# sunbains/scann-rust

Measured on NVIDIA B200. Metric: queries/sec @ recall@10>=0.95 (Tree-AH 10Mx96), higher is better.
Workload: dtype u8 LUT / u32 accumulate, f32 reorder

## Files before the change

scann-rust_b200/csrc/tc_gemm.cu:

```cuda
#include <cuda.h>
#include <cuda_bf16.h>

#include <stdlib.h>

#include <algorithm>

#include "kernels.h"

namespace scann {

namespace {

constexpr int kTcBM = 128;
constexpr int kTcBN = 128;
constexpr int kTcAtomK = 64;
constexpr int kTcAtomBytes = kTcBM * 128;
constexpr int kTcEpiWarps = 16;
constexpr int kTcThreads = 32 * (2 + kTcEpiWarps);
constexpr int kTcTmemCols = 512;
constexpr int kWqLane = 8;
constexpr int kWqFlushAt = 6;
constexpr int kWqBytes = kWqLane * 32 * 8 + 16;

__device__ __forceinline__ uint32_t smem_u32(const void* p) {
// ... 326 lines not shown
  tc_fence_before();
  __syncthreads();
  if (warp == 2) {
    tc_fence_after();
    asm volatile("tcgen05.dealloc.cta_group::1.sync.aligned.b32 %0, %1;" ::"r"(tmem_base), "r"(kTcTmemCols) : "memory");
  }
}

template <bool I8>
__global__ void __launch_bounds__(256) tc_prep_rows_kernel(const void* __restrict__ src, size_t n, size_t dim,
                                                           size_t stride, size_t kpad, size_t rows_pad, float scale,
                                                           int want_norm, __nv_bfloat16* __restrict__ dst,
                                                           float* __restrict__ hx, float* __restrict__ norm_max_key) {
  const size_t r = static_cast<size_t>(blockIdx.x) * 8 + (threadIdx.x >> 5);
  const int lane = threadIdx.x & 31;
  if (r >= rows_pad) return;
  float s = 0.0f;
  for (size_t d = lane; d < kpad; d += 32) {
    float v = 0.0f;
    if (r < n && d < dim)
      v = I8 ? static_cast<float>(static_cast<const int8_t*>(src)[r * stride + d])
             : static_cast<const float*>(src)[r * stride + d];
    dst[r * kpad + d] = __float2bfloat16_rn(v);
    const float f = I8 ? v * scale : v;
    s = fmaf(f, f, s);
  }
#pragma unroll
  for (int o = 16; o > 0; o >>= 1) s += __shfl_xor_sync(0xFFFFFFFFu, s, o);
  if (lane == 0) {
    hx[r] = r < n ? (want_norm ? 0.5f * s : 0.0f) : __int_as_float(0x7F800000);
    if (r < n && norm_max_key) atomicMax(reinterpret_cast<uint32_t*>(norm_max_key), __float_as_uint(s));
  }
}

__global__ void __launch_bounds__(256) tc_prep_queries_kernel(const float* __restrict__ q, size_t nq, size_t dim,
                                                              size_t kpad, size_t q_pad, float scale,
                                                              __nv_bfloat16* __restrict__ dst, float* __restrict__ qn) {
  const size_t r = static_cast<size_t>(blockIdx.x) * 8 + (threadIdx.x >> 5);
  const int lane = threadIdx.x & 31;
  if (r >= q_pad) return;
  float s = 0.0f;
  for (size_t d = lane; d < kpad; d += 32) {
    const float v = (r < nq && d < dim) ? q[r * dim + d] : 0.0f;
    dst[r * kpad + d] = __float2bfloat16_rn(v * scale);
    s = fmaf(v, v, s);
  }
#pragma unroll
  for (int o = 16; o > 0; o >>= 1) s += __shfl_xor_sync(0xFFFFFFFFu, s, o);
  if (lane == 0) qn[r] = s;
}

typedef CUresult (*EncodeTiledFn)(CUtensorMap*, CUtensorMapDataType, cuuint32_t, void*, const cuuint64_t*,
                                  const cuuint64_t*, const cuuint32_t*, const cuuint32_t*, CUtensorMapInterleave,
                                  CUtensorMapSwizzle, CUtensorMapL2promotion, CUtensorMapFloatOOBfill);

EncodeTiledFn encode_fn() {
  static EncodeTiledFn fn = [] {
    void* p = nullptr;
    cudaDriverEntryPointQueryResult qres;
    if (cudaGetDriverEntryPoint("cuTensorMapEncodeTiled", &p, cudaEnableDefault, &qres) != cudaSuccess ||
        qres != cudaDriverEntryPointSuccess)
      p = nullptr;
    return reinterpret_cast<EncodeTiledFn>(p);
  }();
  return fn;
}

scann_status make_map(CUtensorMap* map, const void* base, size_t rows, size_t kpad) {
  EncodeTiledFn fn = encode_fn();
  SCANN_REQUIRE(fn != nullptr, SCANN_UNAVAILABLE, "cuTensorMapEncodeTiled is not available in this driver");
  cuuint64_t dims[2] = {kpad, rows};
  cuuint64_t strides[1] = {kpad * 2};
  cuuint32_t box[2] = {kTcAtomK, kTcBM};
  cuuint32_t estr[2] = {1, 1};
  CUresult r = fn(map, CU_TENSOR_MAP_DATA_TYPE_BFLOAT16, 2, const_cast<void*>(base), dims, strides, box, estr,
                  CU_TENSOR_MAP_INTERLEAVE_NONE, CU_TENSOR_MAP_SWIZZLE_128B, CU_TENSOR_MAP_L2_PROMOTION_L2_256B,
                  CU_TENSOR_MAP_FLOAT_OOB_FILL_NONE);
  SCANN_REQUIRE(r == CUDA_SUCCESS, SCANN_INTERNAL, "cuTensorMapEncodeTiled failed (%d)", static_cast<int>(r));
  return SCANN_OK;
}

}

scann_status tc_make_map_u8(void* map, const void* base, size_t rows, size_t row_bytes) {
  EncodeTiledFn fn = encode_fn();
  SCANN_REQUIRE(fn != nullptr, SCANN_UNAVAILABLE, "cuTensorMapEncodeTiled is not available in this driver");
  cuuint64_t dims[2] = {row_bytes, rows};
  cuuint64_t strides[1] = {row_bytes};
  cuuint32_t box[2] = {128, 128};
  cuuint32_t estr[2] = {1, 1};
  CUresult r = fn(static_cast<CUtensorMap*>(map), CU_TENSOR_MAP_DATA_TYPE_UINT8, 2, const_cast<void*>(base), dims,
                  strides, box, estr, CU_TENSOR_MAP_INTERLEAVE_NONE, CU_TENSOR_MAP_SWIZZLE_128B,
                  CU_TENSOR_MAP_L2_PROMOTION_L2_256B, CU_TENSOR_MAP_FLOAT_OOB_FILL_NONE);
  SCANN_REQUIRE(r == CUDA_SUCCESS, SCANN_INTERNAL, "cuTensorMapEncodeTiled(u8) failed (%d)", static_cast<int>(r));
  return SCANN_OK;
}

namespace {

template <int MT, int KA>
scann_status launch_tc(const CUtensorMap& tmA, const CUtensorMap& tmB, const TcArgs& a, int sms, cudaStream_t s) {
  constexpr int kBudget = 225 * 1024 - kTcEpiWarps * kWqBytes;
  constexpr int kStagesRaw = (kBudget - MT * KA * kTcAtomBytes) / (KA * kTcAtomBytes);
  constexpr int STAGES = kStagesRaw > 6 ? 6 : kStagesRaw;
  static_assert(STAGES >= 2, "operand tiles do not fit");
  const size_t smem = 1024 + static_cast<size_t>(MT + STAGES) * KA * kTcAtomBytes + (2 * STAGES + 6) * 8 + 16 +
                      kTcEpiWarps * kWqBytes;
  auto kern = tc_score_kernel<MT, KA, STAGES>;
  SCANN_CUDA(cudaFuncSetAttribute(kern, cudaFuncAttributeMaxDynamicSharedMemorySize, static_cast<int>(smem)));
  const uint32_t total = a.q_tiles * a.n_units;
  const unsigned grid = static_cast<unsigned>(std::min<uint32_t>(total, static_cast<uint32_t>(sms)));
  kern<<<grid, kTcThreads, smem, s>>>(tmA, tmB, a);
  SCANN_CUDA(cudaGetLastError());
  return SCANN_OK;
}

}

size_t tc_kpad(size_t dim) { return (dim + kTcAtomK - 1) / kTcAtomK * kTcAtomK; }
bool tc_supported(size_t dim) { return dim >= 1 && tc_kpad(dim) <= 256; }
size_t tc_rows_pad(size_t n) { return (n + kTcBN - 1) / kTcBN * kTcBN; }
size_t tc_queries_pad(size_t nq, size_t dim) {
  const size_t m = (tc_kpad(dim) <= 128 ? 2 : 1) * kTcBM;
  return (nq + m - 1) / m * m;
}

scann_status tc_prepare_rows(const void* rows, bool i8, size_t n, size_t dim, size_t stride, float scale,
                             bool want_norm, void* dst_bf16, float* hx, float* norm_max, cudaStream_t s) {
  const size_t kpad = tc_kpad(dim), rows_pad = tc_rows_pad(n);
  if (rows_pad == 0) return SCANN_OK;
  if (norm_max) SCANN_CUDA(cudaMemsetAsync(norm_max, 0, sizeof(float), s));
  const unsigned grid = static_cast<unsigned>((rows_pad + 7) / 8);
  if (i8)
    tc_prep_rows_kernel<true><<<grid, 256, 0, s>>>(rows, n, dim, stride, kpad, rows_pad, scale, want_norm ? 1 : 0,
                                                   static_cast<__nv_bfloat16*>(dst_bf16), hx, norm_max);
  else
    tc_prep_rows_kernel<false><<<grid, 256, 0, s>>>(rows, n, dim, stride, kpad, rows_pad, scale, want_norm ? 1 : 0,
                                                    static_cast<__nv_bfloat16*>(dst_bf16), hx, norm_max);
  SCANN_CUDA(cudaGetLastError());
  return SCANN_OK;
}

scann_status tc_prepare_queries(const float* q, size_t nq, size_t dim, float scale, void* dst_bf16, float* qn,
                                cudaStream_t s) {
  const size_t kpad = tc_kpad(dim), q_pad = tc_queries_pad(nq, dim);
  if (q_pad == 0) return SCANN_OK;
  tc_prep_queries_kernel<<<static_cast<unsigned>((q_pad + 7) / 8), 256, 0, s>>>(
      q, nq, dim, kpad, q_pad, scale, static_cast<__nv_bfloat16*>(dst_bf16), qn);
  SCANN_CUDA(cudaGetLastError());
  return SCANN_OK;
}

scann_status launch_tc_scores(const TcScoreParams& p, cudaStream_t s) {
  SCANN_REQUIRE(tc_supported(p.dim), SCANN_INVALID_ARGUMENT, "dimension %zu too large for the tensor-core path", p.dim);
  SCANN_REQUIRE(p.row0 % kTcBN == 0, SCANN_INTERNAL, "row0 must be a multiple of %d", kTcBN);
  if (p.nq == 0 || p.nrows == 0) return SCANN_OK;
  const size_t kpad = tc_kpad(p.dim);
  const int ka = static_cast<int>(kpad / kTcAtomK);
  const int mt = ka <= 2 ? 2 : 1;
  CUtensorMap tmA, tmB;
  SCANN_TRY(make_map(&tmA, p.q_bf16, tc_queries_pad(p.nq, p.dim), kpad));
  SCANN_TRY(make_map(&tmB, p.rows_bf16, p.rows_pad_total, kpad));
  TcArgs a;
  a.nq = static_cast<uint32_t>(p.nq);
  a.q_tiles = static_cast<uint32_t>(tc_queries_pad(p.nq, p.dim) / (mt * kTcBM));
  a.row0 = static_cast<uint32_t>(p.row0);
  a.n_tiles = static_cast<uint32_t>((p.nrows + kTcBN - 1) / kTcBN);
  a.tile_stride = static_cast<uint32_t>(p.tile_stride < 1 ? 1 : p.tile_stride);
  uint32_t want_units = static_cast<uint32_t>(std::max(1, 4 * p.sms / static_cast<int>(a.q_tiles)));
  uint32_t tpu = (a.n_tiles + want_units - 1) / want_units;
  if (tpu < 8) {
    const uint32_t t8 = std::min<uint32_t>(8, a.n_tiles);
// ... 92 lines not shown
```

scann-rust_b200/csrc/tcscan.cu:

```cuda
#include <cuda.h>

#include <stdlib.h>
#include <string.h>

#include <algorithm>

#include "kernels.h"
#include "lut16_scan_kernel.cuh"
#include "tcscan.h"

namespace scann {

namespace {

constexpr int ts_threads(int EG) { return 32 * (4 + 4 * EG + 8); }
constexpr int kTsRing = 8;
constexpr int kTsHalf = kTsRing / 2;
constexpr int kTsAcol = 256;
constexpr int kTsAtom = 128 * 128;
constexpr uint32_t kTsBig = 32768;
constexpr uint32_t kNoKey = 0xFFFFFFFFu;

__device__ __forceinline__ uint32_t smem_u32(const void* p) {
  return static_cast<uint32_t>(__cvta_generic_to_shared(p));
}
__device__ __forceinline__ void mbar_init(uint32_t bar, uint32_t count) {
  asm volatile("mbarrier.init.shared::cta.b64 [%0], %1;" ::"r"(bar), "r"(count));
}
__device__ __forceinline__ void mbar_expect_tx(uint32_t bar, uint32_t bytes) {
  asm volatile("mbarrier.arrive.expect_tx.shared::cta.b64 _, [%0], %1;" ::"r"(bar), "r"(bytes) : "memory");
}
__device__ __forceinline__ void mbar_arrive(uint32_t bar) {
  asm volatile("mbarrier.arrive.shared::cta.b64 _, [%0];" ::"r"(bar) : "memory");
}
__device__ volatile uint32_t* g_tcs_dbg = nullptr;
__device__ __forceinline__ void dbg_mark(int idx, uint32_t v) {
  volatile uint32_t* d = g_tcs_dbg;
  if (d != nullptr && blockIdx.x == 0) d[8 + idx] = v;
}
__device__ __forceinline__ void mbar_wait(uint32_t bar, uint32_t parity, uint32_t tag = 0) {
  uint32_t ok = 0;
  for (uint32_t it = 0; !ok; ++it) {
    asm volatile(
        "{\n\t.reg .pred p;\n\tmbarrier.try_wait.parity.shared::cta.b64 p, [%1], %2;\n\tselp.u32 %0, 1, 0, p;\n\t}"
        : "=r"(ok)
        : "r"(bar), "r"(parity)
        : "memory");
    if (!ok && it > (1u << 22)) {
      volatile uint32_t* d = g_tcs_dbg;
      if (d != nullptr && atomicCAS(const_cast<uint32_t*>(d), 0u, 1u) == 0u) {
        d[1] = bar;
        d[2] = parity;
        d[3] = tag;
        d[4] = blockIdx.x;
        d[5] = threadIdx.x;
        __threadfence_system();
      }
      __trap();
    }
  }
}
__device__ __forceinline__ void tma_load_2d(uint32_t dst, const CUtensorMap* map, uint32_t bar, int c0, int c1) {
  asm volatile(
      "cp.async.bulk.tensor.2d.shared::cluster.global.mbarrier::complete_tx::bytes [%0], [%1, {%3, %4}], [%2];" ::"r"(dst),
      "l"(map), "r"(bar), "r"(c0), "r"(c1)
      : "memory");
}
__device__ __forceinline__ void tc_fence_before() { asm volatile("tcgen05.fence::before_thread_sync;" ::: "memory"); }
__device__ __forceinline__ void tc_fence_after() { asm volatile("tcgen05.fence::after_thread_sync;" ::: "memory"); }
__device__ __forceinline__ void tc_commit(uint32_t bar) {
  asm volatile("tcgen05.commit.cta_group::1.mbarrier::arrive::one.shared::cluster.b64 [%0];" ::"r"(bar) : "memory");
}
__device__ __forceinline__ void mma_i8_ts(uint32_t d, uint32_t a_tmem, uint64_t bdesc, uint32_t idesc, uint32_t acc) {
  asm volatile(
      "{\n\t.reg .pred p;\n\tsetp.ne.b32 p, %4, 0;\n\t"
      "tcgen05.mma.cta_group::1.kind::i8 [%0], [%1], %2, %3, p;\n\t}" ::"r"(d),
      "r"(a_tmem), "l"(bdesc), "r"(idesc), "r"(acc)
      : "memory");
}
__device__ __forceinline__ void tc_ld32(uint32_t taddr, uint32_t (&v)[32]) {
  asm volatile(
      "tcgen05.ld.sync.aligned.32x32b.x32.b32 "
      "{%0, %1, %2, %3, %4, %5, %6, %7, %8, %9, %10, %11, %12, %13, %14, %15, "
      "%16, %17, %18, %19, %20, %21, %22, %23, %24, %25, %26, %27, %28, %29, %30, %31}, [%32];"
      : "=r"(v[0]), "=r"(v[1]), "=r"(v[2]), "=r"(v[3]), "=r"(v[4]), "=r"(v[5]), "=r"(v[6]), "=r"(v[7]), "=r"(v[8]),
        "=r"(v[9]), "=r"(v[10]), "=r"(v[11]), "=r"(v[12]), "=r"(v[13]), "=r"(v[14]), "=r"(v[15]), "=r"(v[16]),
        "=r"(v[17]), "=r"(v[18]), "=r"(v[19]), "=r"(v[20]), "=r"(v[21]), "=r"(v[22]), "=r"(v[23]), "=r"(v[24]),
        "=r"(v[25]), "=r"(v[26]), "=r"(v[27]), "=r"(v[28]), "=r"(v[29]), "=r"(v[30]), "=r"(v[31])
      : "r"(taddr)
      : "memory");
  asm volatile("tcgen05.wait::ld.sync.aligned;" ::: "memory");
}
__device__ __forceinline__ void tc_ld32_nowait(uint32_t taddr, uint32_t (&v)[32]) {
  asm volatile(
      "tcgen05.ld.sync.aligned.32x32b.x32.b32 "
      "{%0, %1, %2, %3, %4, %5, %6, %7, %8, %9, %10, %11, %12, %13, %14, %15, "
      "%16, %17, %18, %19, %20, %21, %22, %23, %24, %25, %26, %27, %28, %29, %30, %31}, [%32];"
      : "=r"(v[0]), "=r"(v[1]), "=r"(v[2]), "=r"(v[3]), "=r"(v[4]), "=r"(v[5]), "=r"(v[6]), "=r"(v[7]), "=r"(v[8]),
        "=r"(v[9]), "=r"(v[10]), "=r"(v[11]), "=r"(v[12]), "=r"(v[13]), "=r"(v[14]), "=r"(v[15]), "=r"(v[16]),
        "=r"(v[17]), "=r"(v[18]), "=r"(v[19]), "=r"(v[20]), "=r"(v[21]), "=r"(v[22]), "=r"(v[23]), "=r"(v[24]),
        "=r"(v[25]), "=r"(v[26]), "=r"(v[27]), "=r"(v[28]), "=r"(v[29]), "=r"(v[30]), "=r"(v[31])
      : "r"(taddr)
      : "memory");
}
__device__ __forceinline__ void tc_wait_ld() { asm volatile("tcgen05.wait::ld.sync.aligned;" ::: "memory"); }
__device__ __forceinline__ void tc_st32(uint32_t taddr, const uint32_t (&v)[32]) {
  asm volatile(
      "tcgen05.st.sync.aligned.32x32b.x32.b32 [%0], "
      "{%1, %2, %3, %4, %5, %6, %7, %8, %9, %10, %11, %12, %13, %14, %15, %16, "
      "%17, %18, %19, %20, %21, %22, %23, %24, %25, %26, %27, %28, %29, %30, %31, %32};" ::"r"(taddr),
      "r"(v[0]), "r"(v[1]), "r"(v[2]), "r"(v[3]), "r"(v[4]), "r"(v[5]), "r"(v[6]), "r"(v[7]), "r"(v[8]), "r"(v[9]),
      "r"(v[10]), "r"(v[11]), "r"(v[12]), "r"(v[13]), "r"(v[14]), "r"(v[15]), "r"(v[16]), "r"(v[17]), "r"(v[18]),
      "r"(v[19]), "r"(v[20]), "r"(v[21]), "r"(v[22]), "r"(v[23]), "r"(v[24]), "r"(v[25]), "r"(v[26]), "r"(v[27]),
      "r"(v[28]), "r"(v[29]), "r"(v[30]), "r"(v[31])
      : "memory");
}
__device__ __forceinline__ void tc_st8(uint32_t taddr, uint32_t v0) {
  const uint32_t z = 0;
  asm volatile("tcgen05.st.sync.aligned.32x32b.x8.b32 [%0], {%1, %2, %3, %4, %5, %6, %7, %8};" ::"r"(taddr), "r"(v0),
               "r"(z), "r"(z), "r"(z), "r"(z), "r"(z), "r"(z), "r"(z)
               : "memory");
}
__device__ __forceinline__ void tc_wait_st() { asm volatile("tcgen05.wait::st.sync.aligned;" ::: "memory"); }
__device__ __forceinline__ uint64_t umma_desc(uint32_t saddr) {
  return static_cast<uint64_t>((saddr >> 4) & 0x3FFFu) | (1ull << 16) | (64ull << 32) | (1ull << 46) | (2ull << 61);
}
__device__ __forceinline__ uint32_t elect_one() {
  uint32_t pred;
  asm volatile("{\n\t.reg .pred P;\n\telect.sync _|P, 0xFFFFFFFF;\n\tselp.u32 %0, 1, 0, P;\n\t}" : "=r"(pred));
  return pred;
}
__device__ __forceinline__ uint32_t shl_clamp(uint32_t v, uint32_t sh) {
  uint32_t r;
  asm("shl.b32 %0, %1, %2;" : "=r"(r) : "r"(v), "r"(sh));
  return r;
}

struct ExpandMul {
  uint32_t sh[8];
  uint32_t eight;
};
__device__ __forceinline__ void expand_onehot(uint32_t C, uint32_t (&r)[32], const ExpandMul& xm) {
#pragma unroll
  for (int i = 0; i < 8; ++i) {
    uint32_t x, t, t1, t2, t3;
    asm("mul.lo.u32 %0, %1, %2;" : "=r"(x) : "r"(C), "r"(xm.sh[i]));
    const uint32_t nib = x >> 28;
    asm("mul.lo.u32 %0, %1, %2;" : "=r"(t) : "r"(nib), "r"(xm.eight));
    asm("mad.lo.u32 %0, %1, %2, 0xFFFFFFE0;" : "=r"(t1) : "r"(nib), "r"(xm.eight));
    asm("mad.lo.u32 %0, %1, %2, 0xFFFFFFC0;" : "=r"(t2) : "r"(nib), "r"(xm.eight));
    asm("mad.lo.u32 %0, %1, %2, 0xFFFFFFA0;" : "=r"(t3) : "r"(nib), "r"(xm.eight));
    r[4 * i + 0] = shl_clamp(1u, t);
    r[4 * i + 1] = shl_clamp(1u, t1);
    r[4 * i + 2] = shl_clamp(1u, t2);
    r[4 * i + 3] = shl_clamp(1u, t3);
  }
}

__device__ __forceinline__ int score_bound_from_tau(float tau, float mult, float biasS, int smax_all) {
  const float est = __fdiv_rn(__fsub_rn(tau, biasS), mult);
  long long s;
  if (!(est == est)) return -2;
  if (est < -1.0f) s = -1;
  else if (est > static_cast<float>(smax_all)) s = smax_all;
  else s = static_cast<long long>(floorf(est));
  for (int it = 0; it < 8 && s < smax_all && lut16_dequant(static_cast<uint32_t>(s + 1), mult, biasS) <= tau; ++it) ++s;
  for (int it = 0; it < 8 && s >= 0 && lut16_dequant(static_cast<uint32_t>(s), mult, biasS) > tau; --s, ++it) {
  }
  if (s >= 0 && lut16_dequant(static_cast<uint32_t>(s), mult, biasS) > tau) return -2;
  if (s < smax_all && lut16_dequant(static_cast<uint32_t>(s + 1), mult, biasS) <= tau) return -2;
  return static_cast<int>(s);
}

__global__ void tcwl_count_kernel(const uint32_t* __restrict__ tokens, size_t P, uint32_t K, uint32_t L, uint32_t T,
                                  const uint64_t* __restrict__ pt_off, uint32_t* __restrict__ leaf_cnt) {
  const size_t p = static_cast<size_t>(blockIdx.x) * blockDim.x + threadIdx.x;
  if (p >= P || static_cast<uint32_t>(p) % L < T) return;
  const uint32_t leaf = tokens[p];
  if (leaf < K && pt_off[leaf + 1] > pt_off[leaf]) atomicAdd(&leaf_cnt[leaf], 1u);
}

__device__ __forceinline__ void tcwl_entry(uint32_t leaf, const uint32_t* __restrict__ leaf_cnt,
                                           const uint64_t* __restrict__ pt_off, uint32_t& pc, uint32_t& groups,
                                           uint32_t& chunks) {
// ... 4 lines not shown
}

__global__ void __launch_bounds__(1024) tcwl_scan_kernel(const uint32_t* __restrict__ leaf_cnt, uint32_t K,
                                                         const uint32_t* __restrict__ perm,
                                                         const uint64_t* __restrict__ pt_off,
                                                         uint32_t* __restrict__ pair_start,
                                                         uint32_t* __restrict__ group_start,
                                                         uint32_t* __restrict__ item_start,
                                                         uint32_t* __restrict__ counters,
                                                         unsigned long long* __restrict__ pair_points) {
  __shared__ uint32_t s_p[1024], s_g[1024], s_i[1024];
  unsigned long long pp_local = 0;
  const uint32_t per = (K + 1023) / 1024;
  const uint32_t b = threadIdx.x * per, e = min(K, b + per);
  uint32_t sp = 0, sg = 0, si = 0;
  for (uint32_t i = b; i < e; ++i) {
    uint32_t pc, g, c;
    tcwl_entry(perm[i], leaf_cnt, pt_off, pc, g, c);
    sp += pc;
    sg += g;
    si += g * c;
    pp_local += static_cast<unsigned long long>(pc) * (pt_off[perm[i] + 1] - pt_off[perm[i]]);
  }
  if (pair_points && pp_local) atomicAdd(pair_points, pp_local);
  s_p[threadIdx.x] = sp;
  s_g[threadIdx.x] = sg;
  s_i[threadIdx.x] = si;
  __syncthreads();
  for (int o = 1; o < 1024; o <<= 1) {
    uint32_t vp = 0, vg = 0, vi = 0;
    if (threadIdx.x >= o) {
      vp = s_p[threadIdx.x - o];
      vg = s_g[threadIdx.x - o];
      vi = s_i[threadIdx.x - o];
    }
    __syncthreads();
    s_p[threadIdx.x] += vp;
    s_g[threadIdx.x] += vg;
    s_i[threadIdx.x] += vi;
    __syncthreads();
  }
  uint32_t rp = s_p[threadIdx.x] - sp, rg = s_g[threadIdx.x] - sg, ri = s_i[threadIdx.x] - si;
  for (uint32_t i = b; i < e; ++i) {
    const uint32_t leaf = perm[i];
    uint32_t pc, g, c;
    tcwl_entry(leaf, leaf_cnt, pt_off, pc, g, c);
    pair_start[leaf] = rp;
    group_start[leaf] = rg;
    item_start[leaf] = ri;
    rp += pc;
    rg += g;
    ri += g * c;
  }
  if (threadIdx.x == 1023) {
    counters[0] = s_i[1023];
    counters[1] = s_g[1023];
    counters[2] = 0;
  }
}

__global__ void tcwl_scatter_kernel(const uint32_t* __restrict__ tokens, size_t P, uint32_t K, uint32_t L, uint32_t T,
                                    const uint64_t* __restrict__ pt_off, const uint32_t* __restrict__ pair_start,
                                    uint32_t* __restrict__ cursor, uint32_t* __restrict__ sorted_pairs) {
  const size_t p = static_cast<size_t>(blockIdx.x) * blockDim.x + threadIdx.x;
  if (p >= P || static_cast<uint32_t>(p) % L < T) return;
  const uint32_t leaf = tokens[p];
  if (leaf < K && pt_off[leaf + 1] > pt_off[leaf])
    sorted_pairs[pair_start[leaf] + atomicAdd(&cursor[leaf], 1u)] = static_cast<uint32_t>(p);
}

__global__ void tcwl_items_kernel(const uint32_t* __restrict__ leaf_cnt, uint32_t K,
                                  const uint64_t* __restrict__ pt_off, const uint32_t* __restrict__ pair_start,
                                  const uint32_t* __restrict__ group_start, const uint32_t* __restrict__ item_start,
                                  uint4* __restrict__ groups, uint4* __restrict__ items) {
  const uint32_t leaf = blockIdx.x * blockDim.x + threadIdx.x;
  if (leaf >= K) return;
  uint32_t pc, ng, nc;
  tcwl_entry(leaf, leaf_cnt, pt_off, pc, ng, nc);
  if (pc == 0) return;
  const uint32_t tiles = static_cast<uint32_t>((pt_off[leaf + 1] - pt_off[leaf] + kTcsTile - 1) / kTcsTile);
  const uint32_t per = (tiles + nc - 1) / nc;
  const uint32_t pb = pair_start[leaf], gb = group_start[leaf], ib = item_start[leaf];
  for (uint32_t g = 0; g < ng; ++g) {
    groups[gb + g] = make_uint4(leaf, pb + g * kTcsGroup, min(static_cast<uint32_t>(kTcsGroup), pc - g * kTcsGroup), 0u);
    for (uint32_t c = 0; c < nc; ++c)
      items[ib + g * nc + c] = make_uint4(gb + g, c * per, min(tiles, (c + 1) * per), leaf);
  }
}

struct LutArgs {
  const uint4* groups;
  const uint32_t* counters;
  const uint32_t* sorted_pairs;
  const float* queries;
  const float* centers;
  const float* codebook;
  const uint32_t* qthr;
  uint8_t* lut;
  uint4* meta;
  uint32_t* qflag;
  int dim, S, ds, L, use_residuals, row_bytes;
};

__device__ __forceinline__ uint32_t lut16_quantize_nonneg(float v, float mn, float scale) {
  const float y = __fmul_rn(__fsub_rn(v, mn), scale);
  uint32_t i = __float2uint_rd(y);
  i += __fsub_rn(y, __uint2float_rn(i)) >= 0.5f ? 1u : 0u;
  return min(i, 255u);
}

template <int DS>
__global__ void __launch_bounds__(256, DS > 0 ? 4 : 2) tc_lut_kernel(const LutArgs a) {
  extern __shared__ __align__(16) uint8_t sm[];
  const int warp = threadIdx.x >> 5, lane = threadIdx.x & 31;
  float* qres = reinterpret_cast<float*>(sm) + warp * a.dim;
  const int nstep = a.S / 8;
  constexpr int kDs = DS > 0 ? DS : 1;
  float* cbs = reinterpret_cast<float*>(sm) + 8 * a.dim;
  if (DS > 0) {
    for (int i = threadIdx.x; i < a.S * 16 * DS; i += blockDim.x) cbs[i] = __ldg(a.codebook + i);
    __syncthreads();
  }
  const uint32_t ngroups = a.counters[1];
  const uint32_t total = ngroups * kTcsGroup;
  for (uint32_t r = blockIdx.x * 8 + warp; r < total; r += gridDim.x * 8) {
    const uint32_t g = r / kTcsGroup, j = r % kTcsGroup;
    const uint4 G = a.groups[g];
    const uint32_t ncol = (G.z + 15u) & ~15u;
    if (j >= ncol) continue;
    uint8_t* out = a.lut + static_cast<size_t>(r) * a.row_bytes;
    uint32_t val = kTsBig + 1u;
    float mult = 1.0f, biasS = 0.0f;
    uint32_t pair = kNoKey;
    if (j < G.z) {
      pair = a.sorted_pairs[G.y + j];
      const uint32_t q = pair / static_cast<uint32_t>(a.L);
      __syncwarp();
      for (int d = lane; d < a.dim; d += 32) {
        float v = a.queries[static_cast<size_t>(q) * a.dim + d];
        if (a.use_residuals) v = __fsub_rn(v, __ldg(a.centers + static_cast<size_t>(G.x) * a.dim + d));
        qres[d] = v;
      }
      __syncwarp();
      float vals[8][4];
      float mn = 3.402823466e+38f, mx = -3.402823466e+38f;
#pragma unroll
      for (int t = 0; t < 8; ++t) {
        if (t < nstep) {
          const int s = 8 * t + (lane >> 2);
          float cw[4 * kDs];
          if (DS > 0) {
            const float4* c4 = reinterpret_cast<const float4*>(cbs + (128 * t + 4 * lane) * DS);
#pragma unroll
            for (int v = 0; v < kDs; ++v) {
              const float4 x = c4[v];
              cw[4 * v + 0] = x.x;
              cw[4 * v + 1] = x.y;
              cw[4 * v + 2] = x.z;
              cw[4 * v + 3] = x.w;
            }
          }
#pragma unroll
          for (int b = 0; b < 4; ++b) {
            float sum = 0.0f;
            if (DS > 0) {
#pragma unroll
              for (int jj = 0; jj < kDs; ++jj) {
// ... 22 lines not shown
      }
#pragma unroll
      for (int t = 0; t < 8; ++t) {
        if (t < nstep) {
          const uint32_t w = lut16_quantize_nonneg(vals[t][0], mn, scale) | (lut16_quantize_nonneg(vals[t][1], mn, scale) << 8) |
                             (lut16_quantize_nonneg(vals[t][2], mn, scale) << 16) |
                             (lut16_quantize_nonneg(vals[t][3], mn, scale) << 24);
          reinterpret_cast<uint32_t*>(out)[32 * t + lane] = w;
        }
      }
      biasS = __fmul_rn(mn, static_cast<float>(a.S));
      const uint32_t tk = a.qthr[q];
      int sb = -2;
      if (tk != kNoKey) sb = score_bound_from_tau(key_f32(tk), mult, biasS, 255 * a.S);
      if (sb == -2) {
        if (lane == 0) a.qflag[q] = 1u;
      } else {
        val = kTsBig - static_cast<uint32_t>(sb);
      }
    } else {
      for (int v = lane; v < a.S; v += 32) reinterpret_cast<uint4*>(out)[v] = make_uint4(0, 0, 0, 0);
    }
    if (lane < 2) {
      uint4 t = make_uint4(0, 0, 0, 0);
      if (lane == 0) t.x = (val % 255u) | ((val / 255u) << 8);
      reinterpret_cast<uint4*>(out + a.S * 16)[lane] = t;
    }
    if (lane == 0) a.meta[r] = make_uint4(__float_as_uint(mult), __float_as_uint(biasS), val, pair);
  }
}

struct TcsArgs {
  const uint8_t* codes_rm;
  const uint64_t* pt_off;
  const uint4* groups;
  const uint4* items;
  const uint32_t* counters;
  const uint4* meta;
  unsigned long long* qcand;
  uint32_t* qcnt;
  uint32_t* err;
  uint32_t qcap;
  uint32_t nq;
  ExpandMul xm;
  int KA;
  int bpp;
  int L;
};

struct TcsFilter {
  const uint8_t* allow;
  size_t allow_stride;
  const uint32_t* qfilt;
  const uint32_t* blk_off;
  uint32_t num_filters;
};

template <bool FILT>
__device__ __forceinline__ void tcs_emit(const TcsArgs& a, const TcsFilter& f, uint32_t lut_row, uint32_t acc, uint32_t pos,
                                         uint32_t leaf) {
  const uint4 m = __ldg(a.meta + lut_row);
  const uint32_t q = m.w / static_cast<uint32_t>(a.L), rank = m.w - q * static_cast<uint32_t>(a.L);
  if (m.w == kNoKey || q >= a.nq) {
    atomicAdd(a.err, 1u);
    return;
  }
  if (FILT) {
    const uint32_t row = f.qfilt ? __ldg(f.qfilt + q) : 0u;
    if (row >= f.num_filters) return;
    const size_t at = row * f.allow_stride + (static_cast<size_t>(__ldg(f.blk_off + leaf)) + (pos >> 8)) * 32 +
                      ((pos & 255u) >> 3);
    if (!((__ldg(f.allow + at) >> (pos & 7u)) & 1u)) return;
  }
  const uint32_t sum = acc - m.z;
  const float dist = lut16_dequant(sum, __uint_as_float(m.x), __uint_as_float(m.y));
  const uint32_t slot = atomicAdd(a.qcnt + q, 1u);
  if (slot < a.qcap)
    a.qcand[static_cast<size_t>(q) * a.qcap + slot] =
        (static_cast<unsigned long long>(f32_key(dist)) << 32) | (static_cast<unsigned long long>(rank) << 22) | pos;
}

constexpr int kWqCap = 320;
constexpr int kWqStep = 256;

template <int EG, bool FILT>
__global__ void __launch_bounds__(ts_threads(EG), 1) tc_scan_kernel(const __grid_constant__ CUtensorMap tmB, const TcsArgs a,
                                                                    const TcsFilter filt) {
  extern __shared__ uint8_t smem_raw[];
  uint8_t* smem = reinterpret_cast<uint8_t*>((reinterpret_cast<uintptr_t>(smem_raw) + 1023) & ~uintptr_t(1023));
  uint8_t* sB = smem;
  uint64_t* bars = reinterpret_cast<uint64_t*>(sB + (a.KA + 1) * kTsAtom);
  constexpr int kBFull = 0, kBEmpty = 1, kAFull = 2, kAEmpty = 2 + kTsRing, kTFull = 2 + 2 * kTsRing,
                kTEmpty = 4 + 2 * kTsRing, kNumBars = 6 + 2 * kTsRing;
  uint32_t* tmem_slot = reinterpret_cast<uint32_t*>(bars + kNumBars);
  uint4* wq_base = reinterpret_cast<uint4*>(tmem_slot + 4);
  uint32_t* wq_cnt_base = reinterpret_cast<uint32_t*>(wq_base + 8 * kWqCap);
  const int warp = threadIdx.x >> 5, lane = threadIdx.x & 31;
  const uint32_t bar0 = smem_u32(bars);
  auto bar = [&](int i) { return bar0 + 8u * static_cast<uint32_t>(i); };

  if (warp == 0 && lane == 0) asm volatile("prefetch.tensormap [%0];" ::"l"(&tmB) : "memory");
  if (warp == 1 && lane == 0) {
    mbar_init(bar(kBFull), 1);
    mbar_init(bar(kBEmpty), 2);
    for (int i = 0; i < kTsRing; ++i) {
      mbar_init(bar(kAFull + i), 4);
      mbar_init(bar(kAEmpty + i), 1);
    }
    for (int i = 0; i < 2; ++i) {
      mbar_init(bar(kTFull + i), 1);
      mbar_init(bar(kTEmpty + i), 8);
    }
    asm volatile("fence.mbarrier_init.release.cluster;" ::: "memory");
  }
  if (warp == 3) {
    asm volatile("tcgen05.alloc.cta_group::1.sync.aligned.shared::cta.b32 [%0], %1;" ::"r"(smem_u32(tmem_slot)), "r"(512)
                 : "memory");
    asm volatile("tcgen05.relinquish_alloc_permit.cta_group::1.sync.aligned;" ::: "memory");
  }
  tc_fence_before();
  __syncthreads();
  tc_fence_after();
  const uint32_t tmem = *tmem_slot;
  const uint32_t n_items = a.counters[0];
  const int nchunk = a.KA + 1;

  if (warp == 0) {
    if (lane == 0) {
      uint32_t it = 0;
      for (uint32_t item = blockIdx.x; item < n_items; item += gridDim.x, ++it) {
        const uint4 I = a.items[item];
        mbar_wait(bar(kBEmpty), (it & 1u) ^ 1u, 0x100u + it);
        mbar_expect_tx(bar(kBFull), static_cast<uint32_t>(nchunk) * kTsAtom);
        for (int c = 0; c < nchunk; ++c)
          tma_load_2d(smem_u32(sB + c * kTsAtom), &tmB, bar(kBFull), c * 128, static_cast<int>(I.x * kTcsGroup));
      }
    }
  } else if (warp == 1 || warp == 2) {
    const uint32_t pp = warp == 1 ? 0u : 1u;
    if (elect_one()) {
      uint32_t it = 0, ts = 0;
      const uint64_t bd0 = umma_desc(smem_u32(sB));
      const uint32_t d = tmem + pp * kTcsGroup;
      const uint32_t a0 = tmem + kTsAcol + pp * kTsHalf * 32;
      for (uint32_t item = blockIdx.x; item < n_items; item += gridDim.x, ++it) {
        const uint4 I = a.items[item];
        const uint32_t ncol = (a.groups[I.x].z + 15u) & ~15u;
        const uint32_t idesc = (2u << 4) | ((ncol >> 3) << 17) | ((128u >> 4) << 24);
        mbar_wait(bar(kBFull), it & 1u, 0x200u + it);
        for (uint32_t t = I.y; t < I.z; ++t, ++ts) {
          if ((ts & 1u) != pp) continue;
          const uint32_t k = ts >> 1;
          mbar_wait(bar(kTEmpty + pp), (k & 1u) ^ 1u, 0x300000u + ts);
          tc_fence_after();
          uint32_t m = k * static_cast<uint32_t>(nchunk);
          for (int c = 0; c < a.KA; ++c, ++m) {
            const uint32_t sl = m % kTsHalf;
            mbar_wait(bar(kAFull + pp * kTsHalf + sl), (m / kTsHalf) & 1u, 0x400000u + m);
            tc_fence_after();
            const uint64_t bd = bd0 + static_cast<uint64_t>(c) * (kTsAtom >> 4);
            const uint32_t at = a0 + sl * 32;
            mma_i8_ts(d, at, bd, idesc, c != 0 ? 1u : 0u);
            mma_i8_ts(d, at + 8, bd + 2u, idesc, 1u);
            mma_i8_ts(d, at + 16, bd + 4u, idesc, 1u);
            mma_i8_ts(d, at + 24, bd + 6u, idesc, 1u);
            tc_commit(bar(kAEmpty + pp * kTsHalf + sl));
// ... 52 lines not shown
          const uint32_t m = m0 + c;
          if (c < a.KA && (EG == 2 || (m & 1u) == sg)) {
            const uint32_t slot = pp * kTsHalf + (m % kTsHalf);
            uint32_t r[32];
            expand_onehot(w[c], r, a.xm);
            publish();
            mbar_wait(bar(kAEmpty + slot), ((m / kTsHalf) & 1u) ^ 1u, 0x500000u + m);
            tc_fence_after();
            tc_st32(tmem + lane_addr + kTsAcol + slot * 32, r);
            prev_slot = static_cast<int>(slot);
          }
        }
        {
          const uint32_t m = m0 + static_cast<uint32_t>(a.KA);
          if (EG == 2 || (m & 1u) == sg) {
            const uint32_t slot = pp * kTsHalf + (m % kTsHalf);
            publish();
            mbar_wait(bar(kAEmpty + slot), ((m / kTsHalf) & 1u) ^ 1u, 0x600000u + m);
            tc_fence_after();
            tc_st8(tmem + lane_addr + kTsAcol + slot * 32, 0x0000FF01u);
            prev_slot = static_cast<int>(slot);
          }
          publish();
        }
      }
    }
  } else if (warp >= 4 + 4 * EG) {
    const uint32_t ew = static_cast<uint32_t>(warp - (4 + 4 * EG));
    const uint32_t half_id = ew >> 2;
    const uint32_t quad = warp & 3;
    const uint32_t row = quad * 32 + lane;
    const uint32_t lane_addr = (quad * 32) << 16;
    uint4* const wq = wq_base + ew * kWqCap;
    volatile uint32_t* const wq_cnt = wq_cnt_base + ew;
    if (lane == 0) *wq_cnt = 0;
    __syncwarp();
    auto flush = [&]() {
      __syncwarp();
      const uint32_t nw = *wq_cnt;
      for (uint32_t i = lane; i < nw; i += 32) {
        const uint4 e = wq[i];
        tcs_emit<FILT>(a, filt, e.x, e.y, e.z, FILT ? e.w : 0u);
      }
      __syncwarp();
      if (lane == 0) *wq_cnt = 0;
      __syncwarp();
    };
    auto filter32 = [&](const uint32_t (&v)[32], uint32_t c0, uint32_t nlive, bool valid, uint32_t lut_row0, uint32_t p,
                        uint32_t leaf) {
      uint32_t m8[4];
#pragma unroll
      for (int g8 = 0; g8 < 4; ++g8) {
        uint32_t m = v[8 * g8];
#pragma unroll
        for (int j = 1; j < 8; ++j) m = min(m, v[8 * g8 + j]);
        m8[g8] = m;
      }
      if (nlive < 32) m8[2] = m8[3] = kNoKey;
      const uint32_t mall = min(min(m8[0], m8[1]), min(m8[2], m8[3]));
      if (__any_sync(0xFFFFFFFFu, valid && mall <= kTsBig)) {
#pragma unroll
        for (int g8 = 0; g8 < 4; ++g8) {
          const bool hit = valid && m8[g8] <= kTsBig;
          if (__any_sync(0xFFFFFFFFu, hit)) {
            if (*wq_cnt > kWqCap - kWqStep) flush();
            if (hit) {
#pragma unroll
              for (int j = 0; j < 8; ++j)
                if (v[8 * g8 + j] <= kTsBig)
                  wq[atomicAdd(const_cast<uint32_t*>(wq_cnt), 1u)] =
                      make_uint4(lut_row0 + c0 + 8 * g8 + j, v[8 * g8 + j], p, FILT ? leaf : 0u);
            }
            __syncwarp();
          }
        }
      }
    };
    uint32_t ts = 0;
    for (uint32_t item = blockIdx.x; item < n_items; item += gridDim.x) {
      const uint4 I = a.items[item];
      const uint32_t ncol = (a.groups[I.x].z + 15u) & ~15u;
      const uint32_t leaf_n = static_cast<uint32_t>(a.pt_off[I.w + 1] - a.pt_off[I.w]);
      const uint32_t lut_row0 = I.x * kTcsGroup;
      const uint32_t cb = half_id * 64;
      const uint32_t nmine = ncol > cb ? min(64u, ncol - cb) : 0u;
      for (uint32_t t = I.y; t < I.z; ++t, ++ts) {
        const uint32_t as = ts & 1u;
        const uint32_t p = t * kTcsTile + row;
        const bool valid = p < leaf_n;
        mbar_wait(bar(kTFull + as), (ts >> 1) & 1u, 0x700000u + ts);
        tc_fence_after();
        const uint32_t taddr = tmem + lane_addr + as * kTcsGroup + cb;
        uint32_t v0[32];
        if (nmine > 0) {
          tc_ld32_nowait(taddr, v0);
          tc_wait_ld();
        }
        if (nmine <= 32) {
          tc_fence_before();
          __syncwarp();
          if (lane == 0) mbar_arrive(bar(kTEmpty + as));
        }
        if (nmine > 0) filter32(v0, cb, min(32u, nmine), valid, lut_row0, p, I.w);
        if (nmine > 32) {
          tc_ld32_nowait(taddr + 32, v0);
          tc_wait_ld();
          tc_fence_before();
          __syncwarp();
          if (lane == 0) mbar_arrive(bar(kTEmpty + as));
          filter32(v0, cb + 32, nmine - 32, valid, lut_row0, p, I.w);
        }
      }
    }
    flush();
  }

  tc_fence_before();
  __syncthreads();
  if (warp == 3) {
    tc_fence_after();
    asm volatile("tcgen05.dealloc.cta_group::1.sync.aligned.b32 %0, %1;" ::"r"(tmem), "r"(512) : "memory");
  }
}

__global__ void tcs_flag_kernel(const uint32_t* __restrict__ tokens, size_t P, uint32_t L, uint32_t T,
                                const uint32_t* __restrict__ qcnt, uint32_t qcap, uint32_t* __restrict__ qflag,
                                uint32_t* __restrict__ fb_tokens) {
  const size_t p = static_cast<size_t>(blockIdx.x) * blockDim.x + threadIdx.x;
  if (p >= P) return;
  const uint32_t p32 = static_cast<uint32_t>(p);
  const uint32_t q = p32 / L, rank = p32 - q * L;
  const bool f = qflag[q] != 0u || qcnt[q] > qcap;
  fb_tokens[p] = (f && rank >= T) ? tokens[p] : kNoKey;
  if (f && rank == 0) qflag[q] = 1u;
}

__global__ void tcs_debug_kernel(const uint32_t* __restrict__ qcnt, const uint32_t* __restrict__ qflag, size_t nq,
                                 uint32_t qcap, unsigned long long* __restrict__ out ) {
  const size_t q = static_cast<size_t>(blockIdx.x) * blockDim.x + threadIdx.x;
  if (q >= nq) return;
  atomicAdd(&out[0], static_cast<unsigned long long>(qcnt[q]));
  atomicMax(&out[1], static_cast<unsigned long long>(qcnt[q]));
  if (qflag[q]) atomicAdd(&out[2], 1ull);
  if (qcnt[q] > qcap) atomicAdd(&out[3], 1ull);
}

}

bool tc_scan_supported(size_t S, size_t dim) {
  return S >= 8 && S <= 64 && S % 8 == 0 && (S / 8) % 2 == 0 && dim % S == 0 && dim * 4 * 8 + S * 16 * 8 <= 48 * 1024;
}

size_t tc_scan_max_groups(size_t P, size_t K) { return P / kTcsGroup + std::min(K, P) + 1; }

size_t tc_scan_max_items(size_t P, size_t K, size_t max_leaf) {
  const size_t tiles = (max_leaf + kTcsTile - 1) / kTcsTile;
  return tc_scan_max_groups(P, K) * std::max<size_t>(1, (tiles + kTcsItemTiles - 1) / kTcsItemTiles);
}

size_t tc_scan_workspace_bytes(size_t nq, size_t L, size_t K, size_t S, size_t max_leaf, size_t qcap) {
  const size_t P = nq * L, G = tc_scan_max_groups(P, K);
  size_t b = 0;
  auto add = [&](size_t bytes) { b += Workspace::padded(bytes); };
  add(2 * K * 4);
  add(3 * (K + 1) * 4);
  add(16);
  add(P * 4);
  add(G * 16);
  add(tc_scan_max_items(P, K, max_leaf) * 16);
  add(G * kTcsGroup * (S * 16 + 32));
  add(G * kTcsGroup * 16);
  add(nq * qcap * 8);
  add(nq * 4);
  add(nq * 4);
  add(P * 4);
  return b + 4096;
}

scann_status launch_tc_scan(const TcScanParams& p, Workspace& ws, TcScanOut* out, cudaStream_t s) {
  const size_t K = p.K, P = p.nq * p.L, S = p.S;
  const size_t G = tc_scan_max_groups(P, K), I = tc_scan_max_items(P, K, p.max_leaf);
  const int row_bytes = static_cast<int>(S * 16 + 32);
  uint32_t* leaf_cnt = ws.take<uint32_t>(2 * K);
  uint32_t* cursor = leaf_cnt + K;
  uint32_t* starts = ws.take<uint32_t>(3 * (K + 1));
  uint32_t *pair_start = starts, *group_start = starts + (K + 1), *item_start = starts + 2 * (K + 1);
  uint32_t* counters = ws.take<uint32_t>(4);
  uint32_t* sorted_pairs = ws.take<uint32_t>(P);
  uint4* groups = ws.take<uint4>(G);
  uint4* items = ws.take<uint4>(I);
  uint8_t* lut = ws.take<uint8_t>(G * kTcsGroup * row_bytes);
  uint4* meta = ws.take<uint4>(G * kTcsGroup);
  unsigned long long* qcand = ws.take<unsigned long long>(p.nq * p.qcap);
  uint32_t* qcnt = ws.take<uint32_t>(p.nq);
  uint32_t* qflag = ws.take<uint32_t>(p.nq);
  uint32_t* fb_tokens = ws.take<uint32_t>(P);

  const char* dbg_env = getenv("SCANN_TC_DEBUG");
  const bool dbg = dbg_env && dbg_env[0] == '1';
  cudaEvent_t ev[5];
  if (dbg)
    for (auto& e : ev) cudaEventCreate(&e);
  if (dbg) cudaEventRecord(ev[0], s);
  SCANN_CUDA(cudaMemsetAsync(qcnt, 0, p.nq * 4, s));
  SCANN_CUDA(cudaMemsetAsync(qflag, 0, p.nq * 4, s));
  const unsigned pb = static_cast<unsigned>((P + 255) / 256);
  const bool reuse = p.wl_cnt != nullptr && p.wl_pair_start != nullptr && p.wl_sorted_pairs != nullptr;
  const uint32_t* cnt_in = leaf_cnt;
  const uint32_t* pairs_in = sorted_pairs;
  if (reuse) {
    cnt_in = p.wl_cnt;
    pairs_in = p.wl_sorted_pairs;
  } else {
    SCANN_CUDA(cudaMemsetAsync(leaf_cnt, 0, 2 * K * 4, s));
    tcwl_count_kernel<<<pb, 256, 0, s>>>(p.tokens, P, static_cast<uint32_t>(K), static_cast<uint32_t>(p.L),
                                         static_cast<uint32_t>(p.T), p.pt_off, leaf_cnt);
  }
  tcwl_scan_kernel<<<1, 1024, 0, s>>>(cnt_in, static_cast<uint32_t>(K), p.leaf_perm, p.pt_off, pair_start, group_start,
                                      item_start, counters, p.pair_points);
  if (!reuse)
    tcwl_scatter_kernel<<<pb, 256, 0, s>>>(p.tokens, P, static_cast<uint32_t>(K), static_cast<uint32_t>(p.L),
                                           static_cast<uint32_t>(p.T), p.pt_off, pair_start, cursor, sorted_pairs);
  tcwl_items_kernel<<<static_cast<unsigned>((K + 127) / 128), 128, 0, s>>>(cnt_in, static_cast<uint32_t>(K), p.pt_off,
                                                                          reuse ? p.wl_pair_start : pair_start,
                                                                          group_start, item_start, groups, items);
  if (dbg) cudaEventRecord(ev[1], s);
  if (p.ev[0]) cudaEventRecord(p.ev[0], s);
  LutArgs la;
  la.groups = groups;
  la.counters = counters;
  la.sorted_pairs = pairs_in;
  la.queries = p.queries;
  la.centers = p.centers;
  la.codebook = p.codebook;
  la.qthr = p.qthr;
  la.lut = lut;
  la.meta = meta;
  la.qflag = qflag;
  la.dim = static_cast<int>(p.dim);
  la.S = static_cast<int>(S);
  la.ds = static_cast<int>(p.dim / S);
  la.L = static_cast<int>(p.L);
  la.use_residuals = p.use_residuals;
  la.row_bytes = row_bytes;
  const size_t lsm = 8 * p.dim * sizeof(float) + (la.ds <= 2 ? S * 16 * la.ds * sizeof(float) : 0);
  const unsigned lgrid = static_cast<unsigned>(p.sms * (la.ds <= 2 ? 4 : 2));
  if (la.ds == 1) tc_lut_kernel<1><<<lgrid, 256, lsm, s>>>(la);
  else if (la.ds == 2) tc_lut_kernel<2><<<lgrid, 256, lsm, s>>>(la);
  else tc_lut_kernel<0><<<lgrid, 256, lsm, s>>>(la);
  SCANN_CUDA(cudaGetLastError());

  if (dbg) cudaEventRecord(ev[2], s);
  if (p.ev[1]) cudaEventRecord(p.ev[1], s);
  alignas(64) CUtensorMap tmB;
  SCANN_TRY(tc_make_map_u8(&tmB, lut, G * kTcsGroup, static_cast<size_t>(row_bytes)));
  TcsArgs a;
  a.codes_rm = p.codes_rm;
  a.pt_off = p.pt_off;
  a.groups = groups;
  a.items = items;
  a.counters = counters;
  a.meta = meta;
  a.qcand = qcand;
  a.qcnt = qcnt;
  a.qcap = static_cast<uint32_t>(p.qcap);
  a.nq = static_cast<uint32_t>(p.nq);
  a.err = counters + 2;
  for (int i = 0; i < 8; ++i) a.xm.sh[i] = 1u << (28 - 4 * i);
  a.xm.eight = 8u;
  a.KA = static_cast<int>(S / 8);
  a.bpp = static_cast<int>(S / 2);
  a.L = static_cast<int>(p.L);
  TcsFilter tf;
  tf.allow = p.allow;
  tf.allow_stride = p.allow_stride;
  tf.qfilt = p.qfilt;
  tf.blk_off = p.blk_off;
  tf.num_filters = p.num_filters;
  const bool filt = p.allow != nullptr;
  const size_t smem = std::max<size_t>(120 * 1024, 1024 + static_cast<size_t>(a.KA + 1) * kTsAtom + 32 * 8 + 64 +
                                                       8 * kWqCap * 16 + 64);
  const char* eg_env = getenv("SCANN_TC_EXP");
  const bool eg4 = eg_env && eg_env[0] == '4';
  auto kern = eg4 ? (filt ? tc_scan_kernel<4, true> : tc_scan_kernel<4, false>)
                  : (filt ? tc_scan_kernel<2, true> : tc_scan_kernel<2, false>);
  SCANN_CUDA(cudaFuncSetAttribute(kern, cudaFuncAttributeMaxDynamicSharedMemorySize, static_cast<int>(smem)));
  static uint32_t* h_dbg = nullptr;
  if (dbg && h_dbg == nullptr) {
    uint32_t* d_dbg = nullptr;
    if (cudaHostAlloc(&h_dbg, 64 * 4, cudaHostAllocMapped) == cudaSuccess &&
        cudaHostGetDevicePointer(&d_dbg, h_dbg, 0) == cudaSuccess) {
      memset(h_dbg, 0, 64 * 4);
      cudaMemcpyToSymbol(g_tcs_dbg, &d_dbg, sizeof(d_dbg));
    }
  }
  kern<<<p.sms, ts_threads(eg4 ? 4 : 2), smem, s>>>(tmB, a, tf);
  SCANN_CUDA(cudaGetLastError());
  if (dbg) {
    cudaError_t e = cudaStreamSynchronize(s);
    if (e != cudaSuccess && h_dbg)
    {
      fprintf(stderr, "[tcscan] scan kernel failed (%s): timed-out wait = %u, barrier smem 0x%x, parity %u, tag 0x%x, cta %u, thread %u\n",
              cudaGetErrorString(e), h_dbg[0], h_dbg[1], h_dbg[2], h_dbg[3], h_dbg[4], h_dbg[5]);
      fprintf(stderr, "[tcscan] cta 0 progress marks (warp: value):");
      for (int w = 0; w < 14; ++w) fprintf(stderr, " %d:0x%x", w, h_dbg[8 + w]);
      fprintf(stderr, "\n");
    }
  }
  if (dbg) cudaEventRecord(ev[3], s);
  if (p.ev[2]) cudaEventRecord(p.ev[2], s);
  tcs_flag_kernel<<<pb, 256, 0, s>>>(p.tokens, P, static_cast<uint32_t>(p.L), static_cast<uint32_t>(p.T), qcnt,
                                     static_cast<uint32_t>(p.qcap), qflag, fb_tokens);
  SCANN_CUDA(cudaGetLastError());
  if (dbg) {
    cudaEventRecord(ev[4], s);
    unsigned long long* d_st = nullptr;
    unsigned long long st[4] = {0, 0, 0, 0};
    uint32_t cnt[3] = {0, 0, 0};
    cudaMalloc(&d_st, sizeof(st));
    cudaMemsetAsync(d_st, 0, sizeof(st), s);
    tcs_debug_kernel<<<static_cast<unsigned>((p.nq + 255) / 256), 256, 0, s>>>(qcnt, qflag, p.nq,
                                                                              static_cast<uint32_t>(p.qcap), d_st);
    cudaStreamSynchronize(s);
    cudaMemcpy(st, d_st, sizeof(st), cudaMemcpyDeviceToHost);
    cudaMemcpy(cnt, counters, sizeof(cnt), cudaMemcpyDeviceToHost);
    cudaFree(d_st);
    float t[4];
    for (int i = 0; i < 4; ++i) cudaEventElapsedTime(&t[i], ev[i], ev[i + 1]);
    fprintf(stderr,
            "[tcscan] nq=%zu L=%zu items=%u groups=%u | worklist %.3f ms, lut %.3f ms, scan %.3f ms, flag %.3f ms | "
            "candidates/query mean %.1f max %llu (cap %zu), flagged %llu, overflowed %llu, errors %u\n",
            p.nq, p.L, cnt[0], cnt[1], t[0], t[1], t[2], t[3], static_cast<double>(st[0]) / static_cast<double>(p.nq), st[1],
            p.qcap, st[2], st[3], cnt[2]);
    for (auto& e : ev) cudaEventDestroy(e);
  }
  out->qcand = qcand;
  out->qcnt = qcnt;
  out->qflag = qflag;
  out->fb_tokens = fb_tokens;
  out->launches = reuse ? 5 : 7;
  return SCANN_OK;
}

}
```

scann-rust_b200/csrc/tcscan.h:

```cpp
#pragma once

#include "common.cuh"

namespace scann {

constexpr int kTcsTile = 128;
constexpr int kTcsGroup = 128;
constexpr int kTcsItemTiles = 32;

struct TcScanParams {
  const uint32_t* tokens;
  size_t nq, L, K, dim, S;
  size_t T;
  const uint64_t* pt_off;
  const uint32_t* leaf_perm;
  const uint8_t* codes_rm;
  const float* queries;
  const float* centers;
  const float* codebook;
  const uint32_t* qthr;
  int use_residuals;
  size_t max_leaf;
  size_t qcap;
  int sms;
  cudaEvent_t ev[3] = {nullptr, nullptr, nullptr};
  unsigned long long* pair_points = nullptr;
  const uint32_t* wl_cnt = nullptr;
  const uint32_t* wl_pair_start = nullptr;
  const uint32_t* wl_sorted_pairs = nullptr;
  const uint8_t* allow = nullptr;
  size_t allow_stride = 0;
  const uint32_t* qfilt = nullptr;
  uint32_t num_filters = 0;
  const uint32_t* blk_off = nullptr;
};

struct TcScanOut {
  const unsigned long long* qcand;
  const uint32_t* qcnt;
  const uint32_t* qflag;
  const uint32_t* fb_tokens;
  int launches;
};

bool tc_scan_supported(size_t S, size_t dim);
size_t tc_scan_workspace_bytes(size_t nq, size_t L, size_t K, size_t S, size_t max_leaf, size_t qcap);
scann_status launch_tc_scan(const TcScanParams& p, Workspace& ws, TcScanOut* out, cudaStream_t s);
scann_status tc_make_map_u8(void* map, const void* base, size_t rows, size_t row_bytes);

}
```

Measured before the change: 1.585 million.

## Widen tensor-core scan query group to 160 and balance pairs across groups

Raises the number of query-leaf pairs per MMA group from 128 to 160, so each code tile loaded from memory is reused across more queries. This needs a shorter TMEM accumulator ring to stay within the 512-column budget, a tensor map whose box rows are set by the caller, and an epilogue loop that handles 80 columns per half using x16 TMEM loads for the tail. Pairs in a leaf are now split evenly across its groups instead of filling each group to the cap. The costs are a shallower TMEM ring, more shared memory per B tile, and extra epilogue iterations per tile.

```diff
diff --git a/scann-rust_b200/csrc/tc_gemm.cu b/scann-rust_b200/csrc/tc_gemm.cu
--- a/scann-rust_b200/csrc/tc_gemm.cu
+++ b/scann-rust_b200/csrc/tc_gemm.cu
@@ -432,12 +432,12 @@
 
 }
 
-scann_status tc_make_map_u8(void* map, const void* base, size_t rows, size_t row_bytes) {
+scann_status tc_make_map_u8(void* map, const void* base, size_t rows, size_t row_bytes, uint32_t box_rows) {
   EncodeTiledFn fn = encode_fn();
   SCANN_REQUIRE(fn != nullptr, SCANN_UNAVAILABLE, "cuTensorMapEncodeTiled is not available in this driver");
   cuuint64_t dims[2] = {row_bytes, rows};
   cuuint64_t strides[1] = {row_bytes};
-  cuuint32_t box[2] = {128, 128};
+  cuuint32_t box[2] = {128, box_rows};
   cuuint32_t estr[2] = {1, 1};
   CUresult r = fn(static_cast<CUtensorMap*>(map), CU_TENSOR_MAP_DATA_TYPE_UINT8, 2, const_cast<void*>(base), dims,
                   strides, box, estr, CU_TENSOR_MAP_INTERLEAVE_NONE, CU_TENSOR_MAP_SWIZZLE_128B,
diff --git a/scann-rust_b200/csrc/tcscan.cu b/scann-rust_b200/csrc/tcscan.cu
--- a/scann-rust_b200/csrc/tcscan.cu
+++ b/scann-rust_b200/csrc/tcscan.cu
@@ -4,6 +4,7 @@
 #include <string.h>
 
 #include <algorithm>
+#include <vector>
 
 #include "kernels.h"
 #include "lut16_scan_kernel.cuh"
@@ -14,10 +15,12 @@
 namespace {
 
 constexpr int ts_threads(int EG) { return 32 * (4 + 4 * EG + 8); }
-constexpr int kTsRing = 8;
+constexpr int kTsAcol = 2 * kTcsGroup;
+constexpr int kTsRing = (512 - kTsAcol) / 32;
 constexpr int kTsHalf = kTsRing / 2;
-constexpr int kTsAcol = 256;
-constexpr int kTsAtom = 128 * 128;
+static_assert(kTsHalf >= 2 && kTsAcol + 2 * kTsHalf * 32 <= 512, "TMEM budget");
+static_assert(kTcsGroup % 16 == 0 && kTcsGroup <= 256, "MMA N (M = 128) and TMA box rows");
+constexpr int kTsAtom = kTcsGroup * 128;
 constexpr uint32_t kTsBig = 32768;
 constexpr uint32_t kNoKey = 0xFFFFFFFFu;
 
@@ -100,6 +103,15 @@
         "=r"(v[9]), "=r"(v[10]), "=r"(v[11]), "=r"(v[12]), "=r"(v[13]), "=r"(v[14]), "=r"(v[15]), "=r"(v[16]),
         "=r"(v[17]), "=r"(v[18]), "=r"(v[19]), "=r"(v[20]), "=r"(v[21]), "=r"(v[22]), "=r"(v[23]), "=r"(v[24]),
         "=r"(v[25]), "=r"(v[26]), "=r"(v[27]), "=r"(v[28]), "=r"(v[29]), "=r"(v[30]), "=r"(v[31])
+      : "r"(taddr)
+      : "memory");
+}
+__device__ __forceinline__ void tc_ld16_nowait(uint32_t taddr, uint32_t (&v)[32]) {
+  asm volatile(
+      "tcgen05.ld.sync.aligned.32x32b.x16.b32 "
+      "{%0, %1, %2, %3, %4, %5, %6, %7, %8, %9, %10, %11, %12, %13, %14, %15}, [%16];"
+      : "=r"(v[0]), "=r"(v[1]), "=r"(v[2]), "=r"(v[3]), "=r"(v[4]), "=r"(v[5]), "=r"(v[6]), "=r"(v[7]), "=r"(v[8]),
+        "=r"(v[9]), "=r"(v[10]), "=r"(v[11]), "=r"(v[12]), "=r"(v[13]), "=r"(v[14]), "=r"(v[15])
       : "r"(taddr)
       : "memory");
 }
@@ -270,7 +282,9 @@
   const uint32_t per = (tiles + nc - 1) / nc;
   const uint32_t pb = pair_start[leaf], gb = group_start[leaf], ib = item_start[leaf];
   for (uint32_t g = 0; g < ng; ++g) {
-    groups[gb + g] = make_uint4(leaf, pb + g * kTcsGroup, min(static_cast<uint32_t>(kTcsGroup), pc - g * kTcsGroup), 0u);
+    const uint32_t b = static_cast<uint32_t>(static_cast<uint64_t>(g) * pc / ng);
+    const uint32_t e = static_cast<uint32_t>(static_cast<uint64_t>(g + 1) * pc / ng);
+    groups[gb + g] = make_uint4(leaf, pb + b, e - b, 0u);
     for (uint32_t c = 0; c < nc; ++c)
       items[ib + g * nc + c] = make_uint4(gb + g, c * per, min(tiles, (c + 1) * per), leaf);
   }
@@ -459,6 +473,7 @@
 
 constexpr int kWqCap = 320;
 constexpr int kWqStep = 256;
+constexpr uint32_t kEpiCols = kTcsGroup / 2;
 
 template <int EG, bool FILT>
 __global__ void __launch_bounds__(ts_threads(EG), 1) tc_scan_kernel(const __grid_constant__ CUtensorMap tmB, const TcsArgs a,
@@ -677,8 +692,8 @@
       const uint32_t ncol = (a.groups[I.x].z + 15u) & ~15u;
       const uint32_t leaf_n = static_cast<uint32_t>(a.pt_off[I.w + 1] - a.pt_off[I.w]);
       const uint32_t lut_row0 = I.x * kTcsGroup;
-      const uint32_t cb = half_id * 64;
-      const uint32_t nmine = ncol > cb ? min(64u, ncol - cb) : 0u;
+      const uint32_t cb = half_id * kEpiCols;
+      const uint32_t nmine = ncol > cb ? min(kEpiCols, ncol - cb) : 0u;
       for (uint32_t t = I.y; t < I.z; ++t, ++ts) {
         const uint32_t as = ts & 1u;
         const uint32_t p = t * kTcsTile + row;
@@ -686,24 +701,24 @@
         mbar_wait(bar(kTFull + as), (ts >> 1) & 1u, 0x700000u + ts);
         tc_fence_after();
         const uint32_t taddr = tmem + lane_addr + as * kTcsGroup + cb;
-        uint32_t v0[32];
-        if (nmine > 0) {
-          tc_ld32_nowait(taddr, v0);
-          tc_wait_ld();
-        }
-        if (nmine <= 32) {
+        if (nmine == 0) {
           tc_fence_before();
           __syncwarp();
           if (lane == 0) mbar_arrive(bar(kTEmpty + as));
         }
-        if (nmine > 0) filter32(v0, cb, min(32u, nmine), valid, lut_row0, p, I.w);
-        if (nmine > 32) {
-          tc_ld32_nowait(taddr + 32, v0);
+#pragma unroll
+        for (uint32_t c = 0; c < kEpiCols; c += 32) {
+          if (c >= nmine) break;
+          uint32_t v0[32];
+          if (cb + c + 32 <= kTcsGroup) tc_ld32_nowait(taddr + c, v0);
+          else tc_ld16_nowait(taddr + c, v0);
           tc_wait_ld();
-          tc_fence_before();
-          __syncwarp();
-          if (lane == 0) mbar_arrive(bar(kTEmpty + as));
-          filter32(v0, cb + 32, nmine - 32, valid, lut_row0, p, I.w);
+          if (c + 32 >= nmine) {
+            tc_fence_before();
+            __syncwarp();
+            if (lane == 0) mbar_arrive(bar(kTEmpty + as));
+          }
+          filter32(v0, cb + c, min(32u, nmine - c), valid, lut_row0, p, I.w);
         }
       }
     }
@@ -848,7 +863,7 @@
   if (dbg) cudaEventRecord(ev[2], s);
   if (p.ev[1]) cudaEventRecord(p.ev[1], s);
   alignas(64) CUtensorMap tmB;
-  SCANN_TRY(tc_make_map_u8(&tmB, lut, G * kTcsGroup, static_cast<size_t>(row_bytes)));
+  SCANN_TRY(tc_make_map_u8(&tmB, lut, G * kTcsGroup, static_cast<size_t>(row_bytes), kTcsGroup));
   TcsArgs a;
   a.codes_rm = p.codes_rm;
   a.pt_off = p.pt_off;
@@ -873,8 +888,9 @@
   tf.blk_off = p.blk_off;
   tf.num_filters = p.num_filters;
   const bool filt = p.allow != nullptr;
-  const size_t smem = std::max<size_t>(120 * 1024, 1024 + static_cast<size_t>(a.KA + 1) * kTsAtom + 32 * 8 + 64 +
-                                                       8 * kWqCap * 16 + 64);
+  auto scan_smem = [](size_t KA) { return 1024 + (KA + 1) * kTsAtom + 32 * 8 + 64 + 8 * kWqCap * 16 + 64; };
+  static_assert(scan_smem(64 / 8) <= 227 * 1024, "the B tile of the largest S (tc_scan_supported) must fit");
+  const size_t smem = std::max<size_t>(120 * 1024, scan_smem(static_cast<size_t>(a.KA)));
   const char* eg_env = getenv("SCANN_TC_EXP");
   const bool eg4 = eg_env && eg_env[0] == '4';
   auto kern = eg4 ? (filt ? tc_scan_kernel<4, true> : tc_scan_kernel<4, false>)
@@ -920,13 +936,20 @@
     cudaMemcpy(st, d_st, sizeof(st), cudaMemcpyDeviceToHost);
     cudaMemcpy(cnt, counters, sizeof(cnt), cudaMemcpyDeviceToHost);
     cudaFree(d_st);
+    std::vector<uint4> hg(cnt[1]), hi(cnt[0]);
+    cudaMemcpy(hg.data(), groups, hg.size() * sizeof(uint4), cudaMemcpyDeviceToHost);
+    cudaMemcpy(hi.data(), items, hi.size() * sizeof(uint4), cudaMemcpyDeviceToHost);
+    unsigned long long units = 0, grouped = 0;
+    for (const uint4& g : hg) grouped += g.z;
+    for (const uint4& i : hi) units += i.z - i.y;
     float t[4];
     for (int i = 0; i < 4; ++i) cudaEventElapsedTime(&t[i], ev[i], ev[i + 1]);
     fprintf(stderr,
-            "[tcscan] nq=%zu L=%zu items=%u groups=%u | worklist %.3f ms, lut %.3f ms, scan %.3f ms, flag %.3f ms | "
-            "candidates/query mean %.1f max %llu (cap %zu), flagged %llu, overflowed %llu, errors %u\n",
-            p.nq, p.L, cnt[0], cnt[1], t[0], t[1], t[2], t[3], static_cast<double>(st[0]) / static_cast<double>(p.nq), st[1],
-            p.qcap, st[2], st[3], cnt[2]);
+            "[tcscan] nq=%zu L=%zu items=%u groups=%u units=%llu pairs/group %.1f | worklist %.3f ms, lut %.3f ms, "
+            "scan %.3f ms, flag %.3f ms | candidates/query mean %.1f max %llu (cap %zu), flagged %llu, overflowed %llu, "
+            "errors %u\n",
+            p.nq, p.L, cnt[0], cnt[1], units, cnt[1] ? static_cast<double>(grouped) / cnt[1] : 0.0, t[0], t[1], t[2], t[3],
+            static_cast<double>(st[0]) / static_cast<double>(p.nq), st[1], p.qcap, st[2], st[3], cnt[2]);
     for (auto& e : ev) cudaEventDestroy(e);
   }
   out->qcand = qcand;
diff --git a/scann-rust_b200/csrc/tcscan.h b/scann-rust_b200/csrc/tcscan.h
--- a/scann-rust_b200/csrc/tcscan.h
+++ b/scann-rust_b200/csrc/tcscan.h
@@ -5,7 +5,7 @@
 namespace scann {
 
 constexpr int kTcsTile = 128;
-constexpr int kTcsGroup = 128;
+constexpr int kTcsGroup = 160;
 constexpr int kTcsItemTiles = 32;
 
 struct TcScanParams {
@@ -46,6 +46,6 @@
 bool tc_scan_supported(size_t S, size_t dim);
 size_t tc_scan_workspace_bytes(size_t nq, size_t L, size_t K, size_t S, size_t max_leaf, size_t qcap);
 scann_status launch_tc_scan(const TcScanParams& p, Workspace& ws, TcScanOut* out, cudaStream_t s);
-scann_status tc_make_map_u8(void* map, const void* base, size_t rows, size_t row_bytes);
+scann_status tc_make_map_u8(void* map, const void* base, size_t rows, size_t row_bytes, uint32_t box_rows);
 
 }
```

Result: slower. 1.352 million (median of 6 runs) (-14.7%).
